# hpsim/OGL

Hardware: AMD Instinct MI355X
Metric: cg_iters_per_sec (higher is better)
Workload: dtype f64

## Files before the change

### ogl_amd/csrc/device_common.hpp

```cpp
#pragma once
#include "kernels.hpp"

namespace ogl {

namespace {

constexpr int N_WAVES = BLOCK / WAVE;

__device__ __forceinline__ double wave_sum(double v)
{
#pragma unroll
    for (int off = WAVE / 2; off >= 1; off >>= 1) v += __shfl_xor(v, off, WAVE);
    return v;
}

__device__ __forceinline__ double block_sum(double v, double *slot)
{
    v = wave_sum(v);
    const int lane = threadIdx.x & (WAVE - 1), wave = threadIdx.x / WAVE;
    if (lane == 0) slot[wave] = v;
    __syncthreads();
    double s = slot[0];
#pragma unroll
    for (int w = 1; w < N_WAVES; ++w) s += slot[w];
// ... 320 lines not shown
                if ((long)(w * WAVE + lane) + (long)FIN_BLOCK * (k0 + k) < m) s += stage[k * WAVE + lane];
        }
        __syncthreads();
    }
    if (wave == 0) {
        s = wave_sum(s);
        if (lane < LEAD_REPLICAS) {
            const unsigned long long bits = (unsigned long long)__double_as_longlong(s);
            unsigned long long *box = L.box + (size_t)lane * LEAD_REPLICA_STRIDE + array * 2 * FIN_WAVES + 2 * w;
            __hip_atomic_store(box, ((unsigned long long)tag << 32) | (uint32_t)bits, __ATOMIC_RELAXED, LEAD_SCOPE);
            __hip_atomic_store(box + 1, ((unsigned long long)tag << 32) | (uint32_t)(bits >> 32), __ATOMIC_RELAXED, LEAD_SCOPE);
        }
    }
}

__device__ __forceinline__ bool lead_wait(const LeadBox &L, int n_words, uint32_t tag, double *vals, int *timed_out)
{
    if (threadIdx.x == 0) *timed_out = 0;
    __syncthreads();
    if ((int)threadIdx.x < n_words) {
        const unsigned long long *src = L.box + (size_t)(blockIdx.x % LEAD_REPLICAS) * LEAD_REPLICA_STRIDE + threadIdx.x;
        const long long t0 = wall_clock64();
        for (;;) {
            const unsigned long long w = __hip_atomic_load(src, __ATOMIC_RELAXED, LEAD_SCOPE);
            if ((uint32_t)(w >> 32) == tag) {
                reinterpret_cast<uint32_t *>(vals)[threadIdx.x] = (uint32_t)w;
                break;
            }
            if (wall_clock64() - t0 > L.timeout_ticks) {
                *timed_out = 1;
                break;
            }
            __builtin_amdgcn_s_sleep(1);
        }
    }
    __syncthreads();
    return *timed_out == 0;
}
template <int K>
__device__ __forceinline__ void lead_leaders(const LeadBox &L, uint32_t tag, const double *__restrict__ p0,
                                             const double *__restrict__ p1, const double *__restrict__ p2, int m,
                                             double *stage)
{
    if ((int)blockIdx.x < K * FIN_WAVES) {
        const int a = blockIdx.x / FIN_WAVES;
        lead_wave_sums(L, tag, a == 0 ? p0 : (a == 1 ? p1 : p2), m, blockIdx.x % FIN_WAVES, a, stage);
    }
}

__device__ __forceinline__ double lead_total(const double *vals, int a)
{
    double sum = vals[a * FIN_WAVES];
#pragma unroll 1
// ... 91 lines not shown
```

### ogl_amd/csrc/kernels.hpp

```cpp
#pragma once
#include <hip/hip_runtime.h>

#include "common.hpp"

namespace ogl {

struct DevCriterion {
    double tolerance, rel_tol;
    int32_t min_iter, max_iter, frequency, export_res;
};

struct DevScalars {
    double rho, prev_rho, beta;
    double alpha, omega, gamma;
    double norm_factor;
    double init_res, res;
    double xbar;
    double sums[4];
    int32_t iter;
    int32_t stop;
    int32_t n_evals;
    int32_t stop_phase;
    int32_t stop_turn;
    int32_t comm_error;
// ... 295 lines not shown
                      const HaloPutFused *put = nullptr);

void launch_cg_step1x_fin(hipStream_t st, int32_t n, double *p, double *x, const double *r, const double *inv_diag,
                          const DevScalars *sin, DevScalars *sout, const double *part_rho,
                          const double *part_norm, double *history, int first, const LeadBox &lead = LeadBox{},
                          double *p_out = nullptr, const PRing &ring = PRing{});
void launch_cg_step2r_fin(hipStream_t st, int32_t n, double *r, const double *q, const double *inv_diag,
                          double *part_rho, double *part_norm, const DevScalars *sin, DevScalars *sout,
                          const double *part_beta, double *z_out = nullptr,
                          const LeadBox &lead = LeadBox{});
struct HeldZ {
    unsigned long long *tagged = nullptr;
    int32_t grid = 0;
    int32_t x_early = 1;
};
int held_z_grid(int *chunks_per_workgroup);
int launch_resident_census(hipStream_t st, int grid, unsigned *arrived, int *out, long long timeout_ticks);
void launch_cg_step2r1x(hipStream_t st, int32_t n, double *r, const double *q, const double *inv_diag, double *p,
                        double *p_out, double *x, DevScalars *s, const double *part_beta, double *history,
                        const LeadBox &lead, const PRing &ring, const HeldZ &hz);
constexpr int FUSED_FIN_MAX_CHUNKS = 1024;
void launch_cg_turn_sym(hipStream_t st, const DevSym &A, const double *p_in, double *p_out, double *x, const double *z,
                        double *q, double *part_beta, const DevScalars *sin, DevScalars *sout,
                        const double *part_rho, const double *part_norm, double *history, int first,
                        const LeadBox &lead = LeadBox{});
void launch_cg_turn_sym_big(hipStream_t st, const DevSym &A, const double *p_in, double *p_out, double *x,
                            const double *z, double *q, double *part_beta, const DevScalars *s,
                            const HaloFused &hf = HaloFused{}, const double *p_halo_in = nullptr,
                            double *p_halo_out = nullptr);

void launch_gmres_mgs_fold(hipStream_t st, int32_t n, double *w, const double *vprev, double *h_out, const double *vdot,
                           const double *part_in, double *part_out, const DevScalars *gate, const LeadBox &lead = LeadBox{},
                           uint32_t tag = 0);
void launch_bicg_fold1(hipStream_t st, int32_t n, double *p, const double *r, const double *v, const double *inv_diag,
                       double *y, const DevScalars *sin, DevScalars *sout, const double *part_rho,
// ... 115 lines not shown
```

### ogl_amd/csrc/kernels_krylov.hip

```cpp
#include "device_common.hpp"

namespace ogl {

namespace {

__global__ __launch_bounds__(BLOCK) void k_scale(int n, double *__restrict__ v, double f)
{
    const int i = blockIdx.x * BLOCK + threadIdx.x;
    if (i < n) v[i] = v[i] * f;
}

__global__ __launch_bounds__(BLOCK) void k_fill_xbar(int n, double *__restrict__ v,
                                                     const DevScalars *s)
{
    const int i = blockIdx.x * BLOCK + threadIdx.x;
    if (i < n) v[i] = s->xbar;
}

enum PartialOp { P_SUM = 0, P_DOT = 1, P_NORM1 = 2 };
template <int OP>
__global__ __launch_bounds__(BLOCK) void k_partials(int n, int n_chunks,
                                                    const double *__restrict__ a,
                                                    const double *__restrict__ b,
                                                    double *__restrict__ part,
// ... 488 lines not shown
            d += vrh.x * vz.x;
            a += fabs(vrh.x);
        }
        if (rh.n > 1) {
            d += vrh.y * vz.y;
            a += fabs(vrh.y);
        }
        block_sum2(d, a, slot);
        if (threadIdx.x == 0) {
            part_rho[chunk] = d;
            part_norm[chunk] = a;
        }
    }
}

__device__ __forceinline__ void put_tagged(unsigned long long *w, uint32_t tag, double v)
{
    const unsigned long long bits = (unsigned long long)__double_as_longlong(v);
    __hip_atomic_store(w, ((unsigned long long)tag << 32) | (uint32_t)bits, __ATOMIC_RELAXED, LEAD_SCOPE);
    __hip_atomic_store(w + 1, ((unsigned long long)tag << 32) | (uint32_t)(bits >> 32), __ATOMIC_RELAXED, LEAD_SCOPE);
}

__device__ __forceinline__ void lead_wave_sums_tagged(const LeadBox &L, uint32_t tag, const unsigned long long *tagged,
                                                      int m, int w, int array)
{
    constexpr int Q = 4;
    if (threadIdx.x >= WAVE) return;
    const int lane = threadIdx.x;
    const long long t0 = wall_clock64();
    double s = 0.0;
    bool arrived = true;
    for (long i0 = w * WAVE + lane; arrived && i0 < m; i0 += (long)FIN_BLOCK * Q) {
        unsigned long long lo[Q], hi[Q];
        for (;;) {
            bool all = true;
#pragma unroll
            for (int e = 0; e < Q; ++e) {
                const long i = i0 + (long)FIN_BLOCK * e;
                lo[e] = hi[e] = (unsigned long long)tag << 32;
                if (i < m) {
                    lo[e] = __hip_atomic_load(tagged + 4 * i + 2 * array, __ATOMIC_RELAXED, LEAD_SCOPE);
                    hi[e] = __hip_atomic_load(tagged + 4 * i + 2 * array + 1, __ATOMIC_RELAXED, LEAD_SCOPE);
                }
            }
#pragma unroll
            for (int e = 0; e < Q; ++e) all = all && (uint32_t)(lo[e] >> 32) == tag && (uint32_t)(hi[e] >> 32) == tag;
            if (all) break;
            if (wall_clock64() - t0 > L.timeout_ticks) {
                arrived = false;
                break;
            }
            __builtin_amdgcn_s_sleep(1);
        }
#pragma unroll
        for (int e = 0; e < Q; ++e)
            if (i0 + (long)FIN_BLOCK * e < m) s += __longlong_as_double((long long)((hi[e] << 32) | (uint32_t)lo[e]));
    }
    if (!__all(arrived)) return;
    s = wave_sum(s);
    if (lane < LEAD_REPLICAS) put_tagged(L.box + (size_t)lane * LEAD_REPLICA_STRIDE + array * 2 * FIN_WAVES + 2 * w, tag, s);
}

template <int R, int L, int B, int K>
__global__ __launch_bounds__(BLOCK, B) void k_cg_step2r1x(int n, double *__restrict__ r, const double *__restrict__ q,
                                                          const double *__restrict__ inv_diag, double *p, double *p_out,
                                                          double *__restrict__ x, DevScalars *s,
                                                          const double *__restrict__ part_beta,
                                                          unsigned long long *tagged, int n_part, double *history,
                                                          LeadBox lead, const double *p_pend, int ring_phase,
                                                          int x_early)
{
    static_assert(K == 0 || K == 2, "p in place or two p buffers");
    constexpr int D = 2;
    __shared__ double zl[L > 0 ? L * CHUNK_ROWS : 1];
    __shared__ double sh[4];
    __shared__ int sh_stop;
    __shared__ double slot[2 * N_WAVES];
// ... 61 lines not shown
        double d = 0.0, a = 0.0;
        if (rp.n > 0) {
            d += vr.x * vz.x;
            a += fabs(vr.x);
        }
        if (rp.n > 1) {
            d += vr.y * vz.y;
            a += fabs(vr.y);
        }
        block_sum2(d, a, slot);
        if (tx == 0) {
            put_tagged(tagged + 4 * (size_t)chunk, tag, d);
            put_tagged(tagged + 4 * (size_t)chunk + 2, tag, a);
        }
    }
    if (w < 2 * FIN_WAVES) lead_wave_sums_tagged(lead, tag, tagged, n_part, w % FIN_WAVES, w / FIN_WAVES);
    const bool own_term = beta != 0.0;
    const double t_own = own_term ? s_rho / beta : 0.0;
    auto update_x = [&](const RowPair &rp, const double2 &vp, int upto) {
        const bool pend = K > 1 && 1 < upto && ((s_pending >> 1) & 1u);
        if (!pend && !own_term) return;
        double2 vx = ld2_stream(x, rp);
        if (pend) {
            const double2 v1 = ld2(p_pend, rp);
            vx.x += s_t1 * v1.x;
            vx.y += s_t1 * v1.y;
        }
        if (own_term) {
            vx.x += t_own * vp.x;
            vx.y += t_own * vp.y;
        }
        st2_stream(x, rp, vx);
    };
    const bool early = x_early != 0 && !defers;
    if (early) {
#pragma unroll 2
        for (int i = 0; i < mine; ++i) {
            const RowPair rp = my_rows(w + i * G, n);
            update_x(rp, ld2(p, rp), K);
        }
    }
    if (!lead_wait(lead, 4 * FIN_WAVES, tag, lead_words, &lead_timed_out)) {
        if (tx == 0) s->comm_error = s->stop = 1;
        return;
    }
    if (tx == 0) {
        const double prev_rho = s_rho, rho = lead_total(lead_words, 0), norm = lead_total(lead_words, 1);
        int iter = s_iter, n_evals = s_evals, stop = 0;
        double init_res = s_init, res = 0.0;
        bool evaluated = false;
        if (iter > 0 && iter < c_min) {
            iter += 1;
        } else if (iter % c_freq != 0) {
            iter += 1;
        } else {
            evaluated = true;
            n_evals += 1;
// ... 951 lines not shown
constexpr int STEP2R_LEAD_CPW = 2;
void launch_cg_step2r_fin(hipStream_t st, int32_t n, double *r, const double *q, const double *inv_diag,
                          double *part_rho, double *part_norm, const DevScalars *sin, DevScalars *sout,
                          const double *part_beta, double *z_out, const LeadBox &lead)
{
    const int nc = (int)n_chunks(n);
    if (nc == 0) return;
    if (lead.box && nc >= 3 * FIN_WAVES)
        hipLaunchKernelGGL((k_cg_step2r_fin<true, STEP2R_LEAD_CPW>), dim3((nc + STEP2R_LEAD_CPW - 1) / STEP2R_LEAD_CPW),
                           dim3(BLOCK), 0, st, n, r, q, inv_diag, part_rho, part_norm, sin, sout, part_beta, nc, z_out, lead);
    else
        hipLaunchKernelGGL((k_cg_step2r_fin<false, 1>), dim3(nc), dim3(BLOCK), 0, st, n, r, q, inv_diag, part_rho, part_norm,
                           sin, sout, part_beta, nc, z_out, LeadBox{});
}

constexpr int HZ_B = 4, HZ_R = 11, HZ_L = 9;
#define OGL_HELD_Z(K) k_cg_step2r1x<HZ_R, HZ_L, HZ_B, K>

int held_z_grid(int *chunks_per_workgroup)
{
    *chunks_per_workgroup = HZ_R + HZ_L;
    int dev = 0, per_cu[2] = {0, 0};
    hipDeviceProp_t prop;
    if (hipGetDevice(&dev) != hipSuccess || hipGetDeviceProperties(&prop, dev) != hipSuccess) return 0;
    if (hipOccupancyMaxActiveBlocksPerMultiprocessor(&per_cu[0], OGL_HELD_Z(0), BLOCK, 0) != hipSuccess ||
        hipOccupancyMaxActiveBlocksPerMultiprocessor(&per_cu[1], OGL_HELD_Z(2), BLOCK, 0) != hipSuccess)
        return 0;
    return prop.multiProcessorCount * std::min(HZ_B, std::min(per_cu[0], per_cu[1]));
}

int launch_resident_census(hipStream_t st, int grid, unsigned *arrived, int *out, long long timeout_ticks)
{
    hipFuncAttributes fa;
    if (hipFuncGetAttributes(&fa, reinterpret_cast<const void *>(OGL_HELD_Z(2))) != hipSuccess) return 1;
    if (hipMemsetAsync(arrived, 0, sizeof(unsigned), st) != hipSuccess || hipMemsetAsync(out, 0, sizeof(int), st) != hipSuccess)
        return 1;
    hipLaunchKernelGGL((k_resident_census<HZ_B>), dim3(grid), dim3(BLOCK), fa.sharedSizeBytes, st, arrived, out,
                       timeout_ticks);
    return 0;
}

void launch_cg_step2r1x(hipStream_t st, int32_t n, double *r, const double *q, const double *inv_diag, double *p,
                        double *p_out, double *x, DevScalars *s, const double *part_beta, double *history,
                        const LeadBox &lead, const PRing &ring, const HeldZ &hz)
{
    const int nc = (int)n_chunks(n);
    if (nc == 0) return;
    if (ring.k == 2)
        hipLaunchKernelGGL((OGL_HELD_Z(2)), dim3(hz.grid), dim3(BLOCK), 0, st, n, r, q, inv_diag, p, p_out, x, s, part_beta,
                           hz.tagged, nc, history, lead, ring.b[1], ring.phase, hz.x_early);
    else
        hipLaunchKernelGGL((OGL_HELD_Z(0)), dim3(hz.grid), dim3(BLOCK), 0, st, n, r, q, inv_diag, p, p, x, s, part_beta,
// ... 200 lines not shown
```

### ogl_amd/csrc/kernels_spmv_sym.hip

```cpp
#include "device_common.hpp"

namespace ogl {

namespace {

struct SymOffsets {
    int d[SYM_MAX_OFFSETS];
};
template <int MODE, int NDOT, int ND, bool FAST, bool STREAM>
__global__ __launch_bounds__(BLOCK) void k_spmv_sym(int n_rows, int n_chunks, SymOffsets off,
                                                    const uint8_t *__restrict__ mask,
                                                    const double *__restrict__ planes,
                                                    const double *__restrict__ x, const double *__restrict__ b,
                                                    double *__restrict__ y, const double *__restrict__ w,
                                                    double *__restrict__ dot_partials,
                                                    double *__restrict__ dot2_partials, const DevScalars *gate,
                                                    const int *__restrict__ block_order, HaloFused hf)
{
    __shared__ double slot[N_WAVES];
    __shared__ double ys[CHUNK_ROWS];
    if (gate && gate->stop) return;
    const int chunk = block_order ? block_order[blockIdx.x] : xcd_chunk(blockIdx.x);
    if (chunk < 0 || chunk >= n_chunks) return;
    const int t = threadIdx.x;
    const RowPair rp = my_rows(chunk, n_rows);
    const int row = rp.row;
    const unsigned mm = *reinterpret_cast<const unsigned short *>(mask + row);
    const unsigned m0 = mm & 0xffu, m1 = mm >> 8;
    double2 acc;
    acc.x = acc.y = 0.0;
    if (MODE == SPMV_RESIDUAL) acc = ld2(b, rp);
    double2 up[ND];
    const double *own = planes + (long)chunk * (ND * CHUNK_ROWS) + t * ROWS_PER_THREAD;
#pragma unroll
    for (int j = 0; j < ND; ++j)
        up[j] = (STREAM && (j == 0 || (FAST && j == 1))) ? ld_pair_stream(own + (long)j * CHUNK_ROWS)
                                                         : *reinterpret_cast<const double2 *>(own + (long)j * CHUNK_ROWS);
    const double2 xd = ld2(x, rp);
    const int last = n_rows - 1, last_pair = last & ~1;
    double2 lo[ND];
#pragma unroll
    for (int j = 1; j < ND; ++j) {
        const int r0 = max(row - off.d[j], 0), r1 = max(row + 1 - off.d[j], 0);
        const long a0 = (long)(r0 >> 9) * (ND * CHUNK_ROWS) + (long)j * CHUNK_ROWS + (r0 & (CHUNK_ROWS - 1));
        const long a1 = (long)(r1 >> 9) * (ND * CHUNK_ROWS) + (long)j * CHUNK_ROWS + (r1 & (CHUNK_ROWS - 1));
        if (FAST && j >= 2) {
            lo[j] = *reinterpret_cast<const double2 *>(planes + a0);
        } else if (FAST) {
            if (STREAM) {
                lo[j].x = __shfl_up(up[1].y, 1, WAVE);
                if ((t & (WAVE - 1)) == 0) lo[j].x = planes[a0];
            } else {
                lo[j].x = planes[a0];
// ... 41 lines not shown
    if ((m1 >> (ND - 1)) & 1u) {
        const double p = up[0].y * xd.y;
        acc.y = (MODE == SPMV_RESIDUAL) ? acc.y - p : acc.y + p;
    }
#pragma unroll
    for (int j = 1; j < ND; ++j) {
        if ((m0 >> (ND - 1 + j)) & 1u) {
            const double p = up[j].x * xu[j].x;
            acc.x = (MODE == SPMV_RESIDUAL) ? acc.x - p : acc.x + p;
        }
        if ((m1 >> (ND - 1 + j)) & 1u) {
            const double p = up[j].y * xu[j].y;
            acc.y = (MODE == SPMV_RESIDUAL) ? acc.y - p : acc.y + p;
        }
    }
    if (hf.chunk_bptr) halo_fused_add<MODE>(hf, chunk, acc.x, acc.y, ys);
    st2(y, rp, acc);
    if (NDOT >= 1) {
        const double2 vw = ld2(w, rp);
        double d = 0.0, d2 = 0.0;
        if (rp.n > 0) {
            d += vw.x * acc.x;
            d2 += acc.x * acc.x;
        }
        if (rp.n > 1) {
            d += vw.y * acc.y;
            d2 += acc.y * acc.y;
        }
        const double s = block_sum(d, slot);
        if (threadIdx.x == 0) dot_partials[chunk] = s;
// ... 261 lines not shown
    const double rho = s->rho, prev = s->prev_rho;
    const double tmp = (prev == 0.0) ? 0.0 : rho / prev;
    double2 xd;
    double2 acc = turn_sym_rows<ND>(R, m0, m1, tmp, xd);
    st2(p_out, rp, xd);
    if (HALO) {
        __shared__ double ys[CHUNK_ROWS];
        if (hf.chunk_bptr) halo_fused_add<SPMV_PLAIN, true>(hf, chunk, acc.x, acc.y, ys, tmp, ph_in, ph_out);
    }
    st2(q, rp, acc);
    double d = 0.0;
    if (rp.n > 0) d += xd.x * acc.x;
    if (rp.n > 1) d += xd.y * acc.y;
    const double sd = block_sum(d, slot);
    if (threadIdx.x == 0) part_beta[chunk] = sd;
}

}

void launch_spmv_sym(hipStream_t st, const DevSym &A, int mode, const double *x, const double *b, double *y,
                     const SpmvDots &dots, const DevScalars *gate, const HaloFused &hf)
{
    if (A.n_rows == 0) return;
    const int nc = (int)n_chunks(A.n_rows);
    const dim3 grid(A.block_order ? A.n_blocks : xcd_grid(nc)), block(BLOCK);
    SymOffsets off;
    for (int j = 0; j < SYM_MAX_OFFSETS; ++j) off.d[j] = A.d[j];
    bool fast = A.nd >= 2 && A.d[1] == 1;
    for (int j = 2; j < A.nd; ++j) fast = fast && (A.d[j] % 2 == 0);
#define OGL_SYM_K(MODE, NDOT, ND, FAST, STREAM)                                                                          \
// ... 105 lines not shown
        else if (A.stream)                  \
            OGL_TURN_K(ND, false, true);    \
        else                                \
            OGL_TURN_K(ND, false, false);   \
    } while (0)
    if (A.nd == 2)
        OGL_TURN_ND(2);
    else if (A.nd == 3)
        OGL_TURN_ND(3);
    else
        OGL_TURN_ND(4);
#undef OGL_TURN_ND
#undef OGL_TURN_K
}

}
```

### ogl_amd/csrc/launch_key.hpp

```cpp
#pragma once
#include <cstdint>
#include <cstring>
#include <type_traits>

#include "kernels.hpp"

namespace ogl {

struct KeyHasher {
    uint64_t h = 1469598103934665603ull;
    void bytes(const void *p, size_t n)
    {
        const unsigned char *c = static_cast<const unsigned char *>(p);
        for (size_t i = 0; i < n; ++i) h = (h ^ c[i]) * 1099511628211ull;
    }
    template <class T>
    std::enable_if_t<std::is_arithmetic<T>::value || std::is_pointer<T>::value || std::is_enum<T>::value> operator()(const T &v)
    {
        bytes(&v, sizeof(v));
    }
};

#define OGL_VIEW_FIELDS(T, n)                                                                                        \
    static_assert(sizeof(T) == n, "a field of " #T " was added, removed or resized: bring visit(KeyHasher &, const " #T \
// ... 21 lines not shown
{
    h(a.n_rows), h(a.nd);
    for (int j = 0; j < 4; ++j) h(a.d[j]);
    h(a.mask), h(a.planes), h(a.stream), h(a.block_order), h(a.n_blocks);
}
OGL_VIEW_FIELDS(DevSymx, 96);
inline void visit(KeyHasher &h, const DevSymx &a)
{
    h(a.n_rows), h(a.chunks), h(a.chunks_general), h(a.n_blocks_general), h(a.mask), h(a.planes), h(a.ex_rowptr), h(a.ex_cols);
    h(a.ex_lrow), h(a.ex_vals), h(a.stream), h(a.fast), h(a.xcd_group), h(a.n_blocks);
}
OGL_VIEW_FIELDS(LeadBox, 24);
inline void visit(KeyHasher &h, const LeadBox &a) { h(a.box), h(a.timeout_ticks), h(a.early_loads); }
OGL_VIEW_FIELDS(HeldZ, 16);
inline void visit(KeyHasher &h, const HeldZ &a) { h(a.tagged), h(a.grid), h(a.x_early); }

#undef OGL_VIEW_FIELDS

}
```

### ogl_amd/csrc/solver.hpp

```cpp
#pragma once
#include <hip/hip_runtime.h>

#include <algorithm>
#include <map>
#include <memory>
#include <string>
#include <vector>

#include "comm.hpp"
#include "common.hpp"
#include "host_matrix.hpp"
#include "kernels.hpp"
#include "setup_kernels.hpp"
#include "spmv_layouts.hpp"

namespace ogl {

struct MgLevel {
    int32_t n = 0, nnz = 0, n_coarse = 0;
    bool own = true;
    DevBuf<int32_t> row_ptrs, cols;
    DevBuf<double> vals, inv_d;
    DevBuf<int32_t> agg, agg_ptr, agg_rows;
    DevBuf<double> b, xa, xb, t, r, p;
// ... 259 lines not shown
    int run_krylov(ogl_perf *perf);
    struct KrylovRun;
    int krylov_plan(KrylovRun &k);
    int krylov_prepare(KrylovRun &k);
    int krylov_loop(KrylovRun &k);
    int krylov_enqueue(KrylovRun &k, int count);
    int krylov_finish(KrylovRun &k, ogl_perf *perf);
    int gmres_restart(KrylovRun &k, const ogl::DevScalars *gate);
    int gmres_update_x(KrylovRun &k, int cols, const ogl::DevScalars *gate);
    int turn_gmres(KrylovRun &k, int enq, int pe);
    int turn_cg_generic(KrylovRun &k, int enq, int pe);
    int turn_cg_generic_led(KrylovRun &k, int enq, int pe);
    int turn_cg_two_launch(KrylovRun &k, int enq, int pe);
    int turn_cg_three_launch(KrylovRun &k, int enq, int pe);
    int turn_cg_held_z(KrylovRun &k, int enq, int pe);
    int plan_held_z(KrylovRun &k);
    int turn_cg_merged(KrylovRun &k, int enq, int pe);
    int turn_cg_five_launch(KrylovRun &k, int enq, int pe);
    int turn_bicg_folded(KrylovRun &k, int enq, int pe);
    int turn_bicg(KrylovRun &k, int enq, int pe);
    int time_spmv(int repeats, double *avg_ms);
    ogl::DevHalo halo() const;
    double prop(const std::string &key, double dflt) const;
    const ogl_solver *share_from = nullptr;
    const double *offdiag_upper = nullptr, *offdiag_lower = nullptr;
    uint64_t offdiag_sum = 0;
    bool offdiag_valid = false;
    const ogl_label *seen_lower_addr = nullptr, *seen_upper_addr = nullptr;
    ogl_label seen_faces = -1;
    struct SeenIface {
// ... 12 lines not shown
```

### ogl_amd/csrc/solver_krylov.cpp

```cpp
#include "launch_key.hpp"
#include "solver_internal.hpp"

#include <algorithm>
#include <cmath>
#include <cstring>
#include <vector>

using namespace ogl;

HaloPutFused ogl_solver::begin_halo_put()
{
    HaloPutFused put;
    if (!(pat.non_local_nnz > 0 && peer_halo) || prop("haloFused", 1.0) == 0.0 || peer_safe_wait())
        return put;
    if (++halo_seq == 0) ++halo_seq;
    cur_halo = peer_halo_args(halo_seq);
    put.P = cur_halo;
    put.chunk_sptr = d_chunk_sptr.p;
    put.send_pos = d_send_pos.p;
    put.send_idxs = d_send_idxs.p;
    put.ticket = d_ticket.p;
    put.n_put_chunks = n_put_chunks;
    return put;
}
// ... 138 lines not shown
    uint32_t lead_tag = 0;
    DevCriterion crit{};
    bool is_final = false;
    int max_checks = 0, max_turns = 0;
    int prof_stride = 0, prof_cap = 0;
    hipEvent_t ev_chk[2] = {nullptr, nullptr};
    double t_start = 0.0;
    FinArgs fg{}, chk{}, f1{}, f2{};
    const double *beta_ptr = nullptr;
    double *gm = nullptr, *gm_y = nullptr;
    double *y = nullptr, *z = nullptr;
    int enq = 0;
    double *gm_h(int i, int j) const { return gm + (size_t)j * (m + 1) + i; }
    HeldZ hz{};
    bool held_z() const { return hz.grid > 0; }
    PRing ring{};
    double *p_of_turn(int turn) const
    {
        if (ring.k > 0) return ring.b[turn % ring.k];
        return (merged && (turn & 1)) ? p1 : p0;
    }
    PRing ring_of_turn(int turn) const
    {
        PRing r = ring;
        r.phase = ring.k > 0 ? turn % ring.k : 0;
        return r;
    }
    double *p_halo_of_turn(int turn) const { return ph + (size_t)(turn & 1) * n_halo; }
    bool gmres_scale_late() const { return gmres && !generic && has_diag; }
    bool has_diag = false;
// ... 391 lines not shown
    double *p_new = k.p_of_turn(enq + 1);
    if (enq == 0) {
        OGL_HIP_CHECK(hipEventRecord(k.ev_chk[0], st));
        launch_cg_step1x_fin(st, n, k.p_of_turn(0), d_x.p, d_r.p, precond, k.s, k.s2, d_part0.p, d_part1.p, d_history.p, 1,
                             k.lead, p_new, k.ring_of_turn(0));
        OGL_HIP_CHECK(hipEventRecord(k.ev_chk[1], st));
    }
    if (pe >= 0) OGL_HIP_CHECK(hipEventRecord(prof_ev[2 * pe], st));
    OGL_TRY(dist_spmv(SPMV_PLAIN, p_new, nullptr, d_q.p, SpmvDots{p_new, d_part2.p, nullptr}, k.s2));
    if (pe >= 0) OGL_HIP_CHECK(hipEventRecord(prof_ev[2 * pe + 1], st));
    launch_cg_step2r1x(st, n, d_r.p, d_q.p, precond, p_new, k.p_of_turn(enq + 2), d_x.p, k.s2, d_part2.p, d_history.p, k.lead,
                       k.ring_of_turn(enq + 1), k.hz);
    return OGL_OK;
}

int ogl_solver::plan_held_z(KrylovRun &k)
{
    k.hz = HeldZ{};
    props["heldZInUse"] = 0.0;
    props["heldZGridInUse"] = 0.0;
    if (!(k.lead.box != nullptr && k.fused && !k.fused2 && !k.generic && !k.multi && (k.ring.k == 0 || k.ring.k == 2)))
        return OGL_OK;
    bool streams = false;
    switch (spmv_layout) {
    case SpmvLayout::Ell: streams = ell().stream; break;
    case SpmvLayout::Sell: streams = sell().stream; break;
    case SpmvLayout::Sym: streams = sym().stream; break;
    case SpmvLayout::Symx: streams = symx().stream; break;
    default: streams = csr().stream; break;
    }
    if (prop("heldZ", streams ? 1.0 : 0.0) == 0.0 || held_z_census < 0) return OGL_OK;
    int per_wg = 0;
    int grid = held_z_grid(&per_wg);
    grid = std::min(grid, (int)prop("heldZGrid", (double)grid));
    if (grid < 2 * 16) return OGL_OK;
    const double cap = std::min((double)grid * per_wg, prop("heldZMaxChunks", (double)grid * per_wg));
    if ((double)k.nc > cap) return OGL_OK;
    hipStream_t st = k.st;
    const size_t words = 4 * (size_t)k.nc;
    if (!held_z_box || held_z_words < words) {
        ledger::dev_free(held_z_box);
        held_z_box = nullptr;
        void *b = nullptr;
        OGL_HIP_CHECK(ledger::dev_malloc(&b, words * sizeof(unsigned long long), true));
        held_z_box = static_cast<unsigned long long *>(b);
        held_z_words = words;
    }
    OGL_HIP_CHECK(hipMemsetAsync(held_z_box, 0, held_z_words * sizeof(unsigned long long), st));
    if (held_z_census == 0 || held_z_census_grid < grid) {
        void *c = nullptr;
        OGL_HIP_CHECK(ledger::dev_malloc(&c, 2 * sizeof(int)));
        int timed_out = 1;
        const int rc = launch_resident_census(st, grid, static_cast<unsigned *>(c), static_cast<int *>(c) + 1,
                                              (long long)(prop("heldZCensusS", 1.0) * 1e8));
        hipError_t e = rc == 0 ? hipMemcpyAsync(&timed_out, static_cast<int *>(c) + 1, sizeof(int), hipMemcpyDeviceToHost, st)
                               : hipErrorUnknown;
        if (e == hipSuccess) e = hipStreamSynchronize(st);
        ledger::dev_free(c);
        if (e != hipSuccess) return fail(OGL_ERR_HIP, "census of the held-z grid failed: %s", hipGetErrorString(e));
        held_z_census = timed_out ? -1 : 1;
        held_z_census_grid = grid;
        if (timed_out) return OGL_OK;
    }
    k.hz.tagged = held_z_box;
    k.hz.grid = grid;
    k.hz.x_early = prop("heldZEarlyX", 1.0) != 0.0 ? 1 : 0;
    props["heldZInUse"] = 1.0;
    props["heldZGridInUse"] = (double)grid;
    return OGL_OK;
}

int ogl_solver::turn_cg_merged(KrylovRun &k, int enq, int pe)
{
    hipStream_t st = k.st;
    const int n = k.n;
    DevScalars *s = k.s;
    if (pe >= 0) OGL_HIP_CHECK(hipEventRecord(prof_ev[2 * pe], st));
    if (k.merged_halo) {
        launch_cg_turn_sym_big(st, sym(), k.p_of_turn(enq), k.p_of_turn(enq + 1), d_x.p,
                               k.z_kept ? k.z_kept : d_r.p, d_q.p, d_part0.p, s,
                               halo_fused_args(cur_halo), k.p_halo_of_turn(enq), k.p_halo_of_turn(enq + 1));
    } else {
        launch_cg_turn_sym_big(st, sym(), k.p_of_turn(enq), k.p_of_turn(enq + 1), d_x.p,
// ... 99 lines not shown
int ogl_solver::krylov_enqueue(KrylovRun &k, int count)
{
    for (int i = 0; i < count; ++i, ++k.enq) {
        const int enq = k.enq;
        const bool prof = k.prof_stride && enq % k.prof_stride == 0 && enq / k.prof_stride < k.prof_cap;
        const int pe = prof ? enq / k.prof_stride : -1;
        if (k.gmres)
            OGL_TRY(turn_gmres(k, enq, pe));
        else if (k.bicg)
            OGL_TRY(k.bicg_fold ? turn_bicg_folded(k, enq, pe) : turn_bicg(k, enq, pe));
        else if (k.generic)
            OGL_TRY(k.fused ? turn_cg_generic_led(k, enq, pe) : turn_cg_generic(k, enq, pe));
        else if (k.fused2)
            OGL_TRY(turn_cg_two_launch(k, enq, pe));
        else if (k.held_z())
            OGL_TRY(turn_cg_held_z(k, enq, pe));
        else if (k.fused)
            OGL_TRY(turn_cg_three_launch(k, enq, pe));
        else if (k.merged)
            OGL_TRY(turn_cg_merged(k, enq, pe));
        else
            OGL_TRY(turn_cg_five_launch(k, enq, pe));
    }
    return OGL_OK;
}

int ogl_solver::krylov_loop(KrylovRun &k)
{
    hipStream_t st = k.st;
    const bool fused = k.fused;
    auto poll_record = [&](int slot) -> int {
// ... 15 lines not shown
        for (const void *v : {(const void *)d_p.p, (const void *)d_x.p, (const void *)d_r.p, (const void *)d_q.p,
                              (const void *)precond, (const void *)d_part0.p, (const void *)d_part1.p,
                              (const void *)d_part2.p, (const void *)d_history.p, (const void *)d_z.p, (const void *)d_p2.p})
            kh(v);
        for (int i = 0; i < k.ring.k; ++i) kh((const void *)k.ring.b[i]);
        visit(kh, csr());
        switch (spmv_layout) {
        case SpmvLayout::Ell: visit(kh, ell()); break;
        case SpmvLayout::Sell: visit(kh, sell()); break;
        case SpmvLayout::Sym: visit(kh, sym()); break;
        case SpmvLayout::Symx: visit(kh, symx()); break;
        default: break;
        }
        visit(kh, k.lead);
        visit(kh, k.hz);
        const uint64_t key = kh.h;
        if (!cg_graph || key != cg_graph_key) {
            if (cg_graph) {
                (void)hipGraphExecDestroy(cg_graph);
                ledger::destroyed(ledger::GRAPH_EXEC);
            }
            cg_graph = nullptr;
            OGL_HIP_CHECK(hipStreamBeginCapture(st, hipStreamCaptureModeThreadLocal));
            const int before = k.enq;
            const int rc = krylov_enqueue(k, batch);
            k.enq = before;
            hipGraph_t g = nullptr;
            const hipError_t e = hipStreamEndCapture(st, &g);
            if (rc != OGL_OK || e != hipSuccess) {
                if (g) (void)hipGraphDestroy(g);
// ... 211 lines not shown
```

Before: 4657.

## Fuse symmetric SpMV into held-z CG turn as single persistent launch

Adds a persistent 'held-q' CG kernel that computes the symmetric-stencil SpMV in-register and in LDS for each workgroup's chunks. It then performs the residual/preconditioner update, tagged cross-workgroup reductions and the p/x update in the same launch, replacing the separate SpMV turn plus the held-z step kernel. The sym_rows device helper is factored out of k_spmv_sym so both kernels share it. The tagged reduction helper is generalised with a stride so dot partials can live in a six-word box. This trades launch count and intermediate q traffic for higher register and LDS pressure, and it depends on all workgroups being co-resident.

New measurement: 4863 (median of 6 runs). 1.04x the previous value.

```diff
diff --git a/ogl_amd/csrc/device_common.hpp b/ogl_amd/csrc/device_common.hpp
--- a/ogl_amd/csrc/device_common.hpp
+++ b/ogl_amd/csrc/device_common.hpp
@@ -358,12 +358,13 @@
     }
 }
 
-__device__ __forceinline__ bool lead_wait(const LeadBox &L, int n_words, uint32_t tag, double *vals, int *timed_out)
+__device__ __forceinline__ bool lead_wait(const LeadBox &L, int n_words, uint32_t tag, double *vals, int *timed_out,
+                                          int first = 0)
 {
     if (threadIdx.x == 0) *timed_out = 0;
     __syncthreads();
     if ((int)threadIdx.x < n_words) {
-        const unsigned long long *src = L.box + (size_t)(blockIdx.x % LEAD_REPLICAS) * LEAD_REPLICA_STRIDE + threadIdx.x;
+        const unsigned long long *src = L.box + (size_t)(blockIdx.x % LEAD_REPLICAS) * LEAD_REPLICA_STRIDE + first + threadIdx.x;
         const long long t0 = wall_clock64();
         for (;;) {
             const unsigned long long w = __hip_atomic_load(src, __ATOMIC_RELAXED, LEAD_SCOPE);
@@ -381,6 +382,53 @@
     __syncthreads();
     return *timed_out == 0;
 }
+__device__ __forceinline__ void put_tagged(unsigned long long *w, uint32_t tag, double v)
+{
+    const unsigned long long bits = (unsigned long long)__double_as_longlong(v);
+    __hip_atomic_store(w, ((unsigned long long)tag << 32) | (uint32_t)bits, __ATOMIC_RELAXED, LEAD_SCOPE);
+    __hip_atomic_store(w + 1, ((unsigned long long)tag << 32) | (uint32_t)(bits >> 32), __ATOMIC_RELAXED, LEAD_SCOPE);
+}
+
+__device__ __forceinline__ void lead_wave_sums_tagged(const LeadBox &L, uint32_t tag, const unsigned long long *tagged,
+                                                      int stride, int m, int w, int array)
+{
+    constexpr int Q = 4;
+    if (threadIdx.x >= WAVE) return;
+    const int lane = threadIdx.x;
+    const long long t0 = wall_clock64();
+    double s = 0.0;
+    bool arrived = true;
+    for (long i0 = w * WAVE + lane; arrived && i0 < m; i0 += (long)FIN_BLOCK * Q) {
+        unsigned long long lo[Q], hi[Q];
+        for (;;) {
+            bool all = true;
+#pragma unroll
+            for (int e = 0; e < Q; ++e) {
+                const long i = i0 + (long)FIN_BLOCK * e;
+                lo[e] = hi[e] = (unsigned long long)tag << 32;
+                if (i < m) {
+                    lo[e] = __hip_atomic_load(tagged + (size_t)stride * i, __ATOMIC_RELAXED, LEAD_SCOPE);
+                    hi[e] = __hip_atomic_load(tagged + (size_t)stride * i + 1, __ATOMIC_RELAXED, LEAD_SCOPE);
+                }
+            }
+#pragma unroll
+            for (int e = 0; e < Q; ++e) all = all && (uint32_t)(lo[e] >> 32) == tag && (uint32_t)(hi[e] >> 32) == tag;
+            if (all) break;
+            if (wall_clock64() - t0 > L.timeout_ticks) {
+                arrived = false;
+                break;
+            }
+            __builtin_amdgcn_s_sleep(1);
+        }
+#pragma unroll
+        for (int e = 0; e < Q; ++e)
+            if (i0 + (long)FIN_BLOCK * e < m) s += __longlong_as_double((long long)((hi[e] << 32) | (uint32_t)lo[e]));
+    }
+    if (!__all(arrived)) return;
+    s = wave_sum(s);
+    if (lane < LEAD_REPLICAS) put_tagged(L.box + (size_t)lane * LEAD_REPLICA_STRIDE + array * 2 * FIN_WAVES + 2 * w, tag, s);
+}
+
 template <int K>
 __device__ __forceinline__ void lead_leaders(const LeadBox &L, uint32_t tag, const double *__restrict__ p0,
                                              const double *__restrict__ p1, const double *__restrict__ p2, int m,
diff --git a/ogl_amd/csrc/kernels.hpp b/ogl_amd/csrc/kernels.hpp
--- a/ogl_amd/csrc/kernels.hpp
+++ b/ogl_amd/csrc/kernels.hpp
@@ -333,11 +333,21 @@
     int32_t grid = 0;
     int32_t x_early = 1;
 };
+constexpr int HZ_B = 4, HZ_R = 11, HZ_L = 9;
 int held_z_grid(int *chunks_per_workgroup);
 int launch_resident_census(hipStream_t st, int grid, unsigned *arrived, int *out, long long timeout_ticks);
 void launch_cg_step2r1x(hipStream_t st, int32_t n, double *r, const double *q, const double *inv_diag, double *p,
                         double *p_out, double *x, DevScalars *s, const double *part_beta, double *history,
                         const LeadBox &lead, const PRing &ring, const HeldZ &hz);
+struct HeldQ {
+    int32_t on = 0;
+    int32_t n_pos = 0;
+};
+int held_q_positions(const DevSym &A);
+int held_q_occupancy(int *per_cu, size_t *lds_bytes);
+void launch_cg_turn_held_q(hipStream_t st, const DevSym &A, double *r, const double *inv_diag, double *p, double *p_out,
+                           double *x, DevScalars *s, double *history, const LeadBox &lead, const PRing &ring,
+                           const HeldZ &hz, const HeldQ &hq);
 constexpr int FUSED_FIN_MAX_CHUNKS = 1024;
 void launch_cg_turn_sym(hipStream_t st, const DevSym &A, const double *p_in, double *p_out, double *x, const double *z,
                         double *q, double *part_beta, const DevScalars *sin, DevScalars *sout,
diff --git a/ogl_amd/csrc/kernels_krylov.hip b/ogl_amd/csrc/kernels_krylov.hip
--- a/ogl_amd/csrc/kernels_krylov.hip
+++ b/ogl_amd/csrc/kernels_krylov.hip
@@ -526,53 +526,6 @@
     }
 }
 
-__device__ __forceinline__ void put_tagged(unsigned long long *w, uint32_t tag, double v)
-{
-    const unsigned long long bits = (unsigned long long)__double_as_longlong(v);
-    __hip_atomic_store(w, ((unsigned long long)tag << 32) | (uint32_t)bits, __ATOMIC_RELAXED, LEAD_SCOPE);
-    __hip_atomic_store(w + 1, ((unsigned long long)tag << 32) | (uint32_t)(bits >> 32), __ATOMIC_RELAXED, LEAD_SCOPE);
-}
-
-__device__ __forceinline__ void lead_wave_sums_tagged(const LeadBox &L, uint32_t tag, const unsigned long long *tagged,
-                                                      int m, int w, int array)
-{
-    constexpr int Q = 4;
-    if (threadIdx.x >= WAVE) return;
-    const int lane = threadIdx.x;
-    const long long t0 = wall_clock64();
-    double s = 0.0;
-    bool arrived = true;
-    for (long i0 = w * WAVE + lane; arrived && i0 < m; i0 += (long)FIN_BLOCK * Q) {
-        unsigned long long lo[Q], hi[Q];
-        for (;;) {
-            bool all = true;
-#pragma unroll
-            for (int e = 0; e < Q; ++e) {
-                const long i = i0 + (long)FIN_BLOCK * e;
-                lo[e] = hi[e] = (unsigned long long)tag << 32;
-                if (i < m) {
-                    lo[e] = __hip_atomic_load(tagged + 4 * i + 2 * array, __ATOMIC_RELAXED, LEAD_SCOPE);
-                    hi[e] = __hip_atomic_load(tagged + 4 * i + 2 * array + 1, __ATOMIC_RELAXED, LEAD_SCOPE);
-                }
-            }
-#pragma unroll
-            for (int e = 0; e < Q; ++e) all = all && (uint32_t)(lo[e] >> 32) == tag && (uint32_t)(hi[e] >> 32) == tag;
-            if (all) break;
-            if (wall_clock64() - t0 > L.timeout_ticks) {
-                arrived = false;
-                break;
-            }
-            __builtin_amdgcn_s_sleep(1);
-        }
-#pragma unroll
-        for (int e = 0; e < Q; ++e)
-            if (i0 + (long)FIN_BLOCK * e < m) s += __longlong_as_double((long long)((hi[e] << 32) | (uint32_t)lo[e]));
-    }
-    if (!__all(arrived)) return;
-    s = wave_sum(s);
-    if (lane < LEAD_REPLICAS) put_tagged(L.box + (size_t)lane * LEAD_REPLICA_STRIDE + array * 2 * FIN_WAVES + 2 * w, tag, s);
-}
-
 template <int R, int L, int B, int K>
 __global__ __launch_bounds__(BLOCK, B) void k_cg_step2r1x(int n, double *__restrict__ r, const double *__restrict__ q,
                                                           const double *__restrict__ inv_diag, double *p, double *p_out,
@@ -664,7 +617,8 @@
             put_tagged(tagged + 4 * (size_t)chunk + 2, tag, a);
         }
     }
-    if (w < 2 * FIN_WAVES) lead_wave_sums_tagged(lead, tag, tagged, n_part, w % FIN_WAVES, w / FIN_WAVES);
+    if (w < 2 * FIN_WAVES)
+        lead_wave_sums_tagged(lead, tag, tagged + 2 * (w / FIN_WAVES), 4, n_part, w % FIN_WAVES, 1 + w / FIN_WAVES);
     const bool own_term = beta != 0.0;
     const double t_own = own_term ? s_rho / beta : 0.0;
     auto update_x = [&](const RowPair &rp, const double2 &vp, int upto) {
@@ -690,7 +644,7 @@
             update_x(rp, ld2(p, rp), K);
         }
     }
-    if (!lead_wait(lead, 4 * FIN_WAVES, tag, lead_words, &lead_timed_out)) {
+    if (!lead_wait(lead, 4 * FIN_WAVES, tag, lead_words, &lead_timed_out, 2 * FIN_WAVES)) {
         if (tx == 0) s->comm_error = s->stop = 1;
         return;
     }
@@ -1672,7 +1626,6 @@
                            sin, sout, part_beta, nc, z_out, LeadBox{});
 }
 
-constexpr int HZ_B = 4, HZ_R = 11, HZ_L = 9;
 #define OGL_HELD_Z(K) k_cg_step2r1x<HZ_R, HZ_L, HZ_B, K>
 
 int held_z_grid(int *chunks_per_workgroup)
@@ -1684,16 +1637,23 @@
     if (hipOccupancyMaxActiveBlocksPerMultiprocessor(&per_cu[0], OGL_HELD_Z(0), BLOCK, 0) != hipSuccess ||
         hipOccupancyMaxActiveBlocksPerMultiprocessor(&per_cu[1], OGL_HELD_Z(2), BLOCK, 0) != hipSuccess)
         return 0;
-    return prop.multiProcessorCount * std::min(HZ_B, std::min(per_cu[0], per_cu[1]));
+    int per_cu_q = 0;
+    size_t lds_q = 0;
+    if (held_q_occupancy(&per_cu_q, &lds_q) != 0) return 0;
+    return prop.multiProcessorCount * std::min(std::min(HZ_B, per_cu_q), std::min(per_cu[0], per_cu[1]));
 }
 
 int launch_resident_census(hipStream_t st, int grid, unsigned *arrived, int *out, long long timeout_ticks)
 {
     hipFuncAttributes fa;
     if (hipFuncGetAttributes(&fa, reinterpret_cast<const void *>(OGL_HELD_Z(2))) != hipSuccess) return 1;
+    int per_cu_q = 0;
+    size_t lds_q = 0;
+    if (held_q_occupancy(&per_cu_q, &lds_q) != 0) return 1;
+    const size_t lds = std::max((size_t)fa.sharedSizeBytes, lds_q);
     if (hipMemsetAsync(arrived, 0, sizeof(unsigned), st) != hipSuccess || hipMemsetAsync(out, 0, sizeof(int), st) != hipSuccess)
         return 1;
-    hipLaunchKernelGGL((k_resident_census<HZ_B>), dim3(grid), dim3(BLOCK), fa.sharedSizeBytes, st, arrived, out,
+    hipLaunchKernelGGL((k_resident_census<HZ_B>), dim3(grid), dim3(BLOCK), lds, st, arrived, out,
                        timeout_ticks);
     return 0;
 }
diff --git a/ogl_amd/csrc/kernels_spmv_sym.hip b/ogl_amd/csrc/kernels_spmv_sym.hip
--- a/ogl_amd/csrc/kernels_spmv_sym.hip
+++ b/ogl_amd/csrc/kernels_spmv_sym.hip
@@ -1,3 +1,5 @@
+#include <algorithm>
+
 #include "device_common.hpp"
 
 namespace ogl {
@@ -7,23 +9,13 @@
 struct SymOffsets {
     int d[SYM_MAX_OFFSETS];
 };
-template <int MODE, int NDOT, int ND, bool FAST, bool STREAM>
-__global__ __launch_bounds__(BLOCK) void k_spmv_sym(int n_rows, int n_chunks, SymOffsets off,
-                                                    const uint8_t *__restrict__ mask,
-                                                    const double *__restrict__ planes,
-                                                    const double *__restrict__ x, const double *__restrict__ b,
-                                                    double *__restrict__ y, const double *__restrict__ w,
-                                                    double *__restrict__ dot_partials,
-                                                    double *__restrict__ dot2_partials, const DevScalars *gate,
-                                                    const int *__restrict__ block_order, HaloFused hf)
-{
-    __shared__ double slot[N_WAVES];
-    __shared__ double ys[CHUNK_ROWS];
-    if (gate && gate->stop) return;
-    const int chunk = block_order ? block_order[blockIdx.x] : xcd_chunk(blockIdx.x);
-    if (chunk < 0 || chunk >= n_chunks) return;
+template <int MODE, int ND, bool FAST, bool STREAM>
+__device__ __forceinline__ double2 sym_rows(int chunk, const RowPair &rp, int n_rows, const SymOffsets &off,
+                                            const uint8_t *__restrict__ mask, const double *__restrict__ planes,
+                                            const double *__restrict__ x, const double *__restrict__ b,
+                                            double2 &xd_out)
+{
     const int t = threadIdx.x;
-    const RowPair rp = my_rows(chunk, n_rows);
     const int row = rp.row;
     const unsigned mm = *reinterpret_cast<const unsigned short *>(mask + row);
     const unsigned m0 = mm & 0xffu, m1 = mm >> 8;
@@ -36,7 +28,7 @@
     for (int j = 0; j < ND; ++j)
         up[j] = (STREAM && (j == 0 || (FAST && j == 1))) ? ld_pair_stream(own + (long)j * CHUNK_ROWS)
                                                          : *reinterpret_cast<const double2 *>(own + (long)j * CHUNK_ROWS);
-    const double2 xd = ld2(x, rp);
+    const double2 xd = xd_out = ld2(x, rp);
     const int last = n_rows - 1, last_pair = last & ~1;
     double2 lo[ND];
 #pragma unroll
@@ -108,6 +100,27 @@
             acc.y = (MODE == SPMV_RESIDUAL) ? acc.y - p : acc.y + p;
         }
     }
+    return acc;
+}
+
+template <int MODE, int NDOT, int ND, bool FAST, bool STREAM>
+__global__ __launch_bounds__(BLOCK) void k_spmv_sym(int n_rows, int n_chunks, SymOffsets off,
+                                                    const uint8_t *__restrict__ mask,
+                                                    const double *__restrict__ planes,
+                                                    const double *__restrict__ x, const double *__restrict__ b,
+                                                    double *__restrict__ y, const double *__restrict__ w,
+                                                    double *__restrict__ dot_partials,
+                                                    double *__restrict__ dot2_partials, const DevScalars *gate,
+                                                    const int *__restrict__ block_order, HaloFused hf)
+{
+    __shared__ double slot[N_WAVES];
+    __shared__ double ys[CHUNK_ROWS];
+    if (gate && gate->stop) return;
+    const int chunk = block_order ? block_order[blockIdx.x] : xcd_chunk(blockIdx.x);
+    if (chunk < 0 || chunk >= n_chunks) return;
+    const RowPair rp = my_rows(chunk, n_rows);
+    double2 xd;
+    double2 acc = sym_rows<MODE, ND, FAST, STREAM>(chunk, rp, n_rows, off, mask, planes, x, b, xd);
     if (hf.chunk_bptr) halo_fused_add<MODE>(hf, chunk, acc.x, acc.y, ys);
     st2(y, rp, acc);
     if (NDOT >= 1) {
@@ -399,6 +412,240 @@
     if (rp.n > 1) d += xd.y * acc.y;
     const double sd = block_sum(d, slot);
     if (threadIdx.x == 0) part_beta[chunk] = sd;
+}
+
+template <int R, int L, int B, int K, int ND, bool FAST>
+__global__ __launch_bounds__(BLOCK, B) void k_cg_turn_held_q(int n, int n_chunks, int n_pos, SymOffsets off,
+                                                             const uint8_t *__restrict__ mask,
+                                                             const double *__restrict__ planes,
+                                                             const int *__restrict__ block_order, double *__restrict__ r,
+                                                             const double *__restrict__ inv_diag, double *p, double *p_out,
+                                                             double *__restrict__ x, DevScalars *s,
+                                                             unsigned long long *tagged, double *history, LeadBox lead,
+                                                             const double *p_pend, int ring_phase, int x_early)
+{
+    static_assert(K == 0 || K == 2, "p in place or two p buffers");
+    constexpr int D = 2;
+    constexpr int TW = 6;
+    __shared__ double zl[L > 0 ? L * CHUNK_ROWS : 1];
+    __shared__ double sh[4];
+    __shared__ int sh_stop;
+    __shared__ double slot[2 * N_WAVES];
+    __shared__ double lead_words[LEAD_BOX_WORDS / 2];
+    __shared__ int lead_timed_out;
+    const uint32_t seq = s->launch_seq;
+    const int stopped = s->stop;
+    const double s_rho = s->rho, s_nf = s->norm_factor, s_init = s->init_res;
+    const int phase = K > 0 ? ring_phase : 0;
+    const bool defers = K > 0 && phase != 0;
+    const unsigned s_pending = K > 0 ? (unsigned)s->defer_valid : 0u;
+    const double s_t1 = K > 0 ? s->t_ring[1] : 0.0;
+    const int s_iter = s->iter, s_evals = s->n_evals;
+    const double c_tol = s->crit.tolerance, c_rel = s->crit.rel_tol;
+    const int c_min = s->crit.min_iter, c_max = s->crit.max_iter, c_freq = s->crit.frequency, c_exp = s->crit.export_res;
+    const int G = gridDim.x, w = blockIdx.x, tx = threadIdx.x;
+    if (stopped) return;
+    auto chunk_of = [&](int i) -> int {
+        const int pos = w + i * G;
+        if (pos >= n_pos) return -1;
+        const int c = block_order ? block_order[pos] : xcd_chunk(pos);
+        return c < n_chunks ? c : -1;
+    };
+    auto rows_of = [&](int chunk) -> RowPair {
+        if (chunk >= 0) return my_rows(chunk, n);
+        RowPair none;
+        none.row = none.n = 0;
+        return none;
+    };
+    double2 zr[R];
+#pragma unroll
+    for (int i = 0; i < R + L; ++i) {
+        const int chunk = chunk_of(i);
+        if (chunk < 0) continue;
+        const RowPair rp = my_rows(chunk, n);
+        double2 xd;
+        double2 vq = sym_rows<SPMV_PLAIN, ND, FAST, true>(chunk, rp, n, off, mask, planes, p, nullptr, xd);
+        if (rp.n < 2) vq.y = 0.0;
+        if (rp.n < 1) vq.x = 0.0;
+        if (i < R) {
+            zr[i < R ? i : 0] = vq;
+        } else {
+            zl[(i - R) * CHUNK_ROWS + ROWS_PER_THREAD * tx] = vq.x;
+            zl[(i - R) * CHUNK_ROWS + ROWS_PER_THREAD * tx + 1] = vq.y;
+        }
+        double d = 0.0;
+        if (rp.n > 0) d += xd.x * vq.x;
+        if (rp.n > 1) d += xd.y * vq.y;
+        const double sd = block_sum(d, slot);
+        if (tx == 0) put_tagged(tagged + TW * (size_t)chunk, seq, sd);
+    }
+    const int lead0 = G >= 3 * FIN_WAVES ? 2 * FIN_WAVES : 0;
+    if (w >= lead0 && w < lead0 + FIN_WAVES) lead_wave_sums_tagged(lead, seq, tagged, TW, n_chunks, w - lead0, 0);
+    double2 fr[D], fi[D];
+    auto ask = [&](int i, int d) {
+        const RowPair rp = rows_of(chunk_of(i));
+        fr[d] = ld2(r, rp);
+        fi[d].x = fi[d].y = 1.0;
+        if (inv_diag) fi[d] = ld2_stream(inv_diag, rp);
+    };
+#pragma unroll
+    for (int d = 0; d < D; ++d) ask(d, d);
+    if (!lead_wait(lead, 2 * FIN_WAVES, seq, lead_words, &lead_timed_out)) {
+        if (tx == 0) s->comm_error = s->stop = 1;
+        return;
+    }
+    if (tx == 0) sh[0] = lead_total(lead_words, 0);
+    __syncthreads();
+    const double beta = sh[0];
+    const uint32_t tag = seq + 1;
+#pragma unroll
+    for (int i = 0; i < R + L; ++i) {
+        const int chunk = chunk_of(i);
+        if (chunk < 0) {
+            if (i + D < R + L) ask(i + D, i % D);
+            continue;
+        }
+        const RowPair rp = my_rows(chunk, n);
+        double2 vr = fr[i % D];
+        const double2 vi = fi[i % D];
+        if (i + D < R + L) ask(i + D, i % D);
+        double2 vq;
+        if (i < R) {
+            vq = zr[i < R ? i : 0];
+        } else {
+            vq.x = zl[(i - R) * CHUNK_ROWS + ROWS_PER_THREAD * tx];
+            vq.y = zl[(i - R) * CHUNK_ROWS + ROWS_PER_THREAD * tx + 1];
+        }
+        if (beta != 0.0) {
+            const double t = s_rho / beta;
+            vr.x -= t * vq.x;
+            vr.y -= t * vq.y;
+            st2(r, rp, vr);
+        }
+        double2 vz = vr;
+        if (inv_diag) {
+            vz.x = vr.x * vi.x;
+            vz.y = vr.y * vi.y;
+        }
+        if (i < R) {
+            zr[i < R ? i : 0] = vz;
+        } else {
+            zl[(i - R) * CHUNK_ROWS + ROWS_PER_THREAD * tx] = vz.x;
+            zl[(i - R) * CHUNK_ROWS + ROWS_PER_THREAD * tx + 1] = vz.y;
+        }
+        double d = 0.0, a = 0.0;
+        if (rp.n > 0) {
+            d += vr.x * vz.x;
+            a += fabs(vr.x);
+        }
+        if (rp.n > 1) {
+            d += vr.y * vz.y;
+            a += fabs(vr.y);
+        }
+        block_sum2(d, a, slot);
+        if (tx == 0) {
+            put_tagged(tagged + TW * (size_t)chunk + 2, tag, d);
+            put_tagged(tagged + TW * (size_t)chunk + 4, tag, a);
+        }
+    }
+    if (w < 2 * FIN_WAVES)
+        lead_wave_sums_tagged(lead, tag, tagged + 2 + 2 * (w / FIN_WAVES), TW, n_chunks, w % FIN_WAVES, 1 + w / FIN_WAVES);
+    const bool own_term = beta != 0.0;
+    const double t_own = own_term ? s_rho / beta : 0.0;
+    auto update_x = [&](const RowPair &rp, const double2 &vp, int upto) {
+        const bool pend = K > 1 && 1 < upto && ((s_pending >> 1) & 1u);
+        if (!pend && !own_term) return;
+        double2 vx = ld2_stream(x, rp);
+        if (pend) {
+            const double2 v1 = ld2(p_pend, rp);
+            vx.x += s_t1 * v1.x;
+            vx.y += s_t1 * v1.y;
+        }
+        if (own_term) {
+            vx.x += t_own * vp.x;
+            vx.y += t_own * vp.y;
+        }
+        st2_stream(x, rp, vx);
+    };
+    const bool early = x_early != 0 && !defers;
+    if (early) {
+#pragma unroll 2
+        for (int i = 0; i < R + L; ++i) {
+            const int chunk = chunk_of(i);
+            if (chunk < 0) continue;
+            const RowPair rp = my_rows(chunk, n);
+            update_x(rp, ld2(p, rp), K);
+        }
+    }
+    if (!lead_wait(lead, 4 * FIN_WAVES, tag, lead_words, &lead_timed_out, 2 * FIN_WAVES)) {
+        if (tx == 0) s->comm_error = s->stop = 1;
+        return;
+    }
+    if (tx == 0) {
+        const double prev_rho = s_rho, rho = lead_total(lead_words, 0), norm = lead_total(lead_words, 1);
+        int iter = s_iter, n_evals = s_evals, stop = 0;
+        double init_res = s_init, res = 0.0;
+        bool evaluated = false;
+        if (iter > 0 && iter < c_min) {
+            iter += 1;
+        } else if (iter % c_freq != 0) {
+            iter += 1;
+        } else {
+            evaluated = true;
+            n_evals += 1;
+            res = norm;
+            if (iter == 0) init_res = res / s_nf;
+            res /= s_nf;
+            if (c_exp && history && w == 0) history[iter] = res;
+            if (iter >= c_max) stop = 1;
+            if (res < c_tol) stop = 1;
+            if (c_rel > 0 && res < c_rel * init_res) stop = 1;
+            iter += 1;
+        }
+        sh[1] = prev_rho;
+        sh[2] = rho;
+        sh_stop = stop;
+        if (w == 0) {
+            s->beta = beta;
+            s->prev_rho = prev_rho;
+            s->rho = rho;
+            s->iter = iter;
+            s->x_pending = 0;
+            if (evaluated) {
+                s->n_evals = n_evals;
+                s->init_res = init_res;
+                s->res = res;
+            }
+            if (stop) s->stop = 1;
+            s->launch_seq = seq + 2;
+            s->defer_valid = (defers && !stop) ? (int)(s_pending | (own_term ? 1u << phase : 0u)) : 0;
+            if (defers && own_term) s->t_ring[phase] = t_own;
+        }
+    }
+    __syncthreads();
+    const double prev = sh[1], rho = sh[2];
+    const int stop = sh_stop;
+    const double tmp = (prev == 0.0) ? 0.0 : rho / prev;
+#pragma unroll
+    for (int i = 0; i < R + L; ++i) {
+        const int chunk = chunk_of(i);
+        if (chunk < 0) continue;
+        const RowPair rp = my_rows(chunk, n);
+        double2 vp = ld2(p, rp);
+        if (!defers && !early) update_x(rp, vp, K);
+        if (defers && stop) update_x(rp, vp, phase);
+        if (stop) continue;
+        double2 vz;
+        if (i < R) {
+            vz = zr[i < R ? i : 0];
+        } else {
+            vz.x = zl[(i - R) * CHUNK_ROWS + ROWS_PER_THREAD * tx];
+            vz.y = zl[(i - R) * CHUNK_ROWS + ROWS_PER_THREAD * tx + 1];
+        }
+        vp.x = vz.x + tmp * vp.x;
+        vp.y = vz.y + tmp * vp.y;
+        st2(p_out, rp, vp);
+    }
 }
 
 }
@@ -534,4 +781,75 @@
 #undef OGL_TURN_K
 }
 
-}
+#define OGL_HELD_Q(K, ND, FAST) k_cg_turn_held_q<HZ_R, HZ_L, HZ_B, K, ND, FAST>
+#define OGL_HELD_Q_EACH(DO) \
+    DO(0, 2, false) DO(0, 2, true) DO(0, 3, false) DO(0, 3, true) DO(0, 4, false) DO(0, 4, true) \
+    DO(2, 2, false) DO(2, 2, true) DO(2, 3, false) DO(2, 3, true) DO(2, 4, false) DO(2, 4, true)
+int held_q_positions(const DevSym &A)
+{
+    return A.block_order ? A.n_blocks : xcd_grid((int)n_chunks(A.n_rows));
+}
+
+int held_q_occupancy(int *per_cu, size_t *lds_bytes)
+{
+    *per_cu = HZ_B;
+    *lds_bytes = 0;
+#define OGL_HELD_Q_ASK(K, ND, FAST)                                                                                  \
+    {                                                                                                                \
+        int o = 0;                                                                                                   \
+        hipFuncAttributes fa;                                                                                        \
+        if (hipOccupancyMaxActiveBlocksPerMultiprocessor(&o, OGL_HELD_Q(K, ND, FAST), BLOCK, 0) != hipSuccess ||     \
+            hipFuncGetAttributes(&fa, reinterpret_cast<const void *>(OGL_HELD_Q(K, ND, FAST))) != hipSuccess)        \
+            return 1;                                                                                                \
+        *per_cu = std::min(*per_cu, o);                                                                              \
+        *lds_bytes = std::max(*lds_bytes, (size_t)fa.sharedSizeBytes);                                               \
+    }
+    OGL_HELD_Q_EACH(OGL_HELD_Q_ASK)
+#undef OGL_HELD_Q_ASK
+    return 0;
+}
+
+void launch_cg_turn_held_q(hipStream_t st, const DevSym &A, double *r, const double *inv_diag, double *p, double *p_out,
+                           double *x, DevScalars *s, double *history, const LeadBox &lead, const PRing &ring,
+                           const HeldZ &hz, const HeldQ &hq)
+{
+    if (A.n_rows == 0) return;
+    const int nc = (int)n_chunks(A.n_rows);
+    const dim3 grid(hz.grid), block(BLOCK);
+    SymOffsets off;
+    for (int j = 0; j < SYM_MAX_OFFSETS; ++j) off.d[j] = A.d[j];
+    bool fast = A.nd >= 2 && A.d[1] == 1;
+    for (int j = 2; j < A.nd; ++j) fast = fast && (A.d[j] % 2 == 0);
+#define OGL_HELD_Q_K(K, ND, FAST)                                                                                        \
+    hipLaunchKernelGGL((OGL_HELD_Q(K, ND, FAST)), grid, block, 0, st, A.n_rows, nc, hq.n_pos, off, A.mask, A.planes,     \
+                       A.block_order, r, inv_diag, p, K == 2 ? p_out : p, x, s, hz.tagged, history, lead,                \
+                       K == 2 ? (const double *)ring.b[1] : nullptr, K == 2 ? ring.phase : 0, hz.x_early)
+#define OGL_HELD_Q_ND(K, ND)              \
+    do {                                  \
+        if (fast)                         \
+            OGL_HELD_Q_K(K, ND, true);    \
+        else                              \
+            OGL_HELD_Q_K(K, ND, false);   \
+    } while (0)
+#define OGL_HELD_Q_RING(ND)         \
+    do {                            \
+        if (ring.k == 2)            \
+            OGL_HELD_Q_ND(2, ND);   \
+        else                        \
+            OGL_HELD_Q_ND(0, ND);   \
+    } while (0)
+    static_assert(SYM_MAX_OFFSETS == 4, "instantiations above");
+    if (A.nd == 2)
+        OGL_HELD_Q_RING(2);
+    else if (A.nd == 3)
+        OGL_HELD_Q_RING(3);
+    else
+        OGL_HELD_Q_RING(4);
+#undef OGL_HELD_Q_RING
+#undef OGL_HELD_Q_ND
+#undef OGL_HELD_Q_K
+}
+#undef OGL_HELD_Q_EACH
+#undef OGL_HELD_Q
+
+}
diff --git a/ogl_amd/csrc/launch_key.hpp b/ogl_amd/csrc/launch_key.hpp
--- a/ogl_amd/csrc/launch_key.hpp
+++ b/ogl_amd/csrc/launch_key.hpp
@@ -59,6 +59,8 @@
 inline void visit(KeyHasher &h, const LeadBox &a) { h(a.box), h(a.timeout_ticks), h(a.early_loads); }
 OGL_VIEW_FIELDS(HeldZ, 16);
 inline void visit(KeyHasher &h, const HeldZ &a) { h(a.tagged), h(a.grid), h(a.x_early); }
+OGL_VIEW_FIELDS(HeldQ, 8);
+inline void visit(KeyHasher &h, const HeldQ &a) { h(a.on), h(a.n_pos); }
 
 #undef OGL_VIEW_FIELDS
 
diff --git a/ogl_amd/csrc/solver.hpp b/ogl_amd/csrc/solver.hpp
--- a/ogl_amd/csrc/solver.hpp
+++ b/ogl_amd/csrc/solver.hpp
@@ -297,6 +297,7 @@
     int turn_cg_two_launch(KrylovRun &k, int enq, int pe);
     int turn_cg_three_launch(KrylovRun &k, int enq, int pe);
     int turn_cg_held_z(KrylovRun &k, int enq, int pe);
+    int turn_cg_held_q(KrylovRun &k, int enq, int pe);
     int plan_held_z(KrylovRun &k);
     int turn_cg_merged(KrylovRun &k, int enq, int pe);
     int turn_cg_five_launch(KrylovRun &k, int enq, int pe);
diff --git a/ogl_amd/csrc/solver_krylov.cpp b/ogl_amd/csrc/solver_krylov.cpp
--- a/ogl_amd/csrc/solver_krylov.cpp
+++ b/ogl_amd/csrc/solver_krylov.cpp
@@ -176,6 +176,7 @@
     double *gm_h(int i, int j) const { return gm + (size_t)j * (m + 1) + i; }
     HeldZ hz{};
     bool held_z() const { return hz.grid > 0; }
+    HeldQ hq{};
     PRing ring{};
     double *p_of_turn(int turn) const
     {
@@ -597,9 +598,27 @@
     return OGL_OK;
 }
 
+int ogl_solver::turn_cg_held_q(KrylovRun &k, int enq, int pe)
+{
+    if (pe >= 0) return turn_cg_held_z(k, enq, pe);
+    hipStream_t st = k.st;
+    double *p_new = k.p_of_turn(enq + 1);
+    if (enq == 0) {
+        OGL_HIP_CHECK(hipEventRecord(k.ev_chk[0], st));
+        launch_cg_step1x_fin(st, k.n, k.p_of_turn(0), d_x.p, d_r.p, precond, k.s, k.s2, d_part0.p, d_part1.p, d_history.p, 1,
+                             k.lead, p_new, k.ring_of_turn(0));
+        OGL_HIP_CHECK(hipEventRecord(k.ev_chk[1], st));
+    }
+    launch_cg_turn_held_q(st, sym(), d_r.p, precond, p_new, k.p_of_turn(enq + 2), d_x.p, k.s2, d_history.p, k.lead,
+                          k.ring_of_turn(enq + 1), k.hz, k.hq);
+    return OGL_OK;
+}
+
 int ogl_solver::plan_held_z(KrylovRun &k)
 {
     k.hz = HeldZ{};
+    k.hq = HeldQ{};
+    props["heldQInUse"] = 0.0;
     props["heldZInUse"] = 0.0;
     props["heldZGridInUse"] = 0.0;
     if (!(k.lead.box != nullptr && k.fused && !k.fused2 && !k.generic && !k.multi && (k.ring.k == 0 || k.ring.k == 2)))
@@ -619,8 +638,14 @@
     if (grid < 2 * 16) return OGL_OK;
     const double cap = std::min((double)grid * per_wg, prop("heldZMaxChunks", (double)grid * per_wg));
     if ((double)k.nc > cap) return OGL_OK;
-    hipStream_t st = k.st;
-    const size_t words = 4 * (size_t)k.nc;
+    bool held_q = false;
+    int n_pos = 0;
+    if (spmv_layout == SpmvLayout::Sym) {
+        n_pos = held_q_positions(sym());
+        held_q = prop("heldQ", sym().stream && grid % 8 == 0 ? 1.0 : 0.0) != 0.0 && (double)n_pos <= (double)grid * per_wg;
+    }
+    hipStream_t st = k.st;
+    const size_t words = (held_q ? 6 : 4) * (size_t)k.nc;
     if (!held_z_box || held_z_words < words) {
         ledger::dev_free(held_z_box);
         held_z_box = nullptr;
@@ -650,6 +675,11 @@
     k.hz.x_early = prop("heldZEarlyX", 1.0) != 0.0 ? 1 : 0;
     props["heldZInUse"] = 1.0;
     props["heldZGridInUse"] = (double)grid;
+    if (held_q) {
+        k.hq.on = 1;
+        k.hq.n_pos = n_pos;
+        props["heldQInUse"] = 1.0;
+    }
     return OGL_OK;
 }
 
@@ -779,7 +809,7 @@
         else if (k.fused2)
             OGL_TRY(turn_cg_two_launch(k, enq, pe));
         else if (k.held_z())
-            OGL_TRY(turn_cg_held_z(k, enq, pe));
+            OGL_TRY(k.hq.on ? turn_cg_held_q(k, enq, pe) : turn_cg_held_z(k, enq, pe));
         else if (k.fused)
             OGL_TRY(turn_cg_three_launch(k, enq, pe));
         else if (k.merged)
@@ -825,6 +855,7 @@
         }
         visit(kh, k.lead);
         visit(kh, k.hz);
+        visit(kh, k.hq);
         const uint64_t key = kh.h;
         if (!cg_graph || key != cg_graph_key) {
             if (cg_graph) {
```
